# msaad00/agent-bom

Measured on AMD Instinct MI355X. Metric: findings/sec, higher is better.
Workload: dtype fp32; 1 GPU; model=estate-blast-pipeline, global_batch=327063, seq_len=10000000, parallelism=single, nodes_global=11350000, edges_global=18551093, arena_windows=2000000

## Files before the change

agentbom_amd/graph/gpu_engine.py:

```python

from __future__ import annotations

from typing import Optional

import numpy as np

from agentbom_amd.models.blast import HOP_RISK_FACTORS
from agentbom_amd.models.cwe_impact import (
    IMPACT_CODE,
    IMPACT_CREDENTIAL_ACCESS,
    IMPACT_CODE_EXECUTION,
    IMPACT_DATA_LEAK,
    IMPACT_FILE_ACCESS,
    IMPACT_INJECTION,
    IMPACT_SSRF,
)
from agentbom_amd.scan.synth import ET_CONTAINS, ET_HAS_CRED, ET_PROVIDES_TOOL, ET_USES, SyntheticEstate

_FULL_CRED = {IMPACT_CODE[c] for c in (IMPACT_CODE_EXECUTION, IMPACT_CREDENTIAL_ACCESS,
                                       IMPACT_DATA_LEAK, IMPACT_FILE_ACCESS, IMPACT_SSRF)}
_DB_CRED = {IMPACT_CODE[IMPACT_INJECTION]}
_FULL_TOOL = _FULL_CRED
_DB_TOOL = {IMPACT_CODE[IMPACT_INJECTION]}

# ... 179 lines not shown
        raise ValueError("agent index exceeds int32 offsets")
    agent_off = torch.zeros(n_agents + 1, dtype=torch.int64, device=dev)
    torch.cumsum(torch.bincount(key >> 32, minlength=n_agents), 0, out=agent_off[1:])
    return {
        "agent_off": agent_off.to(torch.int32).contiguous(),
        "agent_srv": (key & 0xFFFFFFFF).to(torch.int32).contiguous(),
    }


def blast_index_enabled() -> bool:
    import os

    return os.environ.get("AGENT_BOM_BLAST_INDEX", "1") != "0"


def match_by_window_enabled() -> bool:
    import os

    return os.environ.get("AGENT_BOM_MATCH_BY_WINDOW", "1") != "0"


def findings_native_enabled() -> bool:
    import os

    return os.environ.get("AGENT_BOM_FINDINGS_NATIVE", "1") != "0"


def findings_ahead_enabled() -> bool:
    import os

    return os.environ.get("AGENT_BOM_FINDINGS_AHEAD", "1") != "0"


def expand_dedup_matches(torch, layout: dict, su, sw):
    dev = su.device
    if su.numel() == 0:
        e = torch.empty(0, dtype=torch.int64, device=dev)
        return e, e.clone()
    run_off = layout["run_off"]
    cnt = run_off[su + 1] - run_off[su]
    rep = torch.repeat_interleave(
        torch.arange(su.numel(), device=dev), cnt)
    ends = torch.cumsum(cnt, 0)
    base = torch.cat([torch.zeros(1, dtype=torch.int64, device=dev), ends[:-1]])
    within = torch.arange(int(ends[-1].item()) if ends.numel() else 0,
                          device=dev) - base[rep]
    rows2 = run_off[su][rep] + within
    orig = layout["perm2"][rows2]
    packed = (orig << 32) | sw[rep]
    packed, _ = torch.sort(packed)
    return (packed >> 32), (packed & 0xFFFFFFFF)



_RANK_WS: dict = {}


def rank_order(torch, scores):
    n = scores.numel()
    if n == 0:
        return torch.empty(0, dtype=torch.int64, device=scores.device)
    if scores.is_cuda:
        from agentbom_amd.ops import native

        return native.rank_bucket_order(scores.contiguous(), _RANK_WS)
    q = (scores * 100).round().clamp(0, 1000).to(torch.int64)
# ... 286 lines not shown

    def _blast_counts_join(self, uniq_pkgs):
        torch = self.torch
        n_up = uniq_pkgs.numel()
        pos = torch.arange(n_up, device=self.device)

        srv, carry = self._expand(self.rev, uniq_pkgs, pos, ET_CONTAINS)
        n_servers = self._distinct_counts(carry, srv, n_up)

        ag, carry2 = self._expand(self.rev, srv, carry, ET_USES)
        n_agents = self._distinct_counts(carry2, ag, n_up)

        cr, carry3 = self._expand(self.fwd, srv, carry, ET_HAS_CRED)
        n_creds_all, n_creds_db = self._distinct_counts(
            carry3, cr, n_up, weights=self.node_is_db_cred
        )
        tl, carry4 = self._expand(self.fwd, srv, carry, ET_PROVIDES_TOOL)
        n_tools_all, n_tools_db = self._distinct_counts(
            carry4, tl, n_up, weights=self.node_is_db_tool
        )
        return {
            "uniq_pkgs": uniq_pkgs,
            "n_servers": n_servers,
            "n_agents": n_agents,
            "n_creds_all": n_creds_all,
            "n_creds_db": n_creds_db,
            "n_tools_all": n_tools_all,
            "n_tools_db": n_tools_db,
        }

    def step(self, blast_depth: int = 1, reach_dist=None):
        torch = self.torch
        assembled = None
        if self.use_gpu:
            from agentbom_amd.ops import native

            if self._match_stream is None:
                self._match_stream = torch.cuda.Stream(device=self.device)
            side = self._match_stream
            if reach_dist is None:
                self._reach_begin()
            side.wait_stream(torch.cuda.current_stream())
            dd = self.match_dedup
            with torch.cuda.stream(side):
                if (dd is not None and self.match_table is not None
                        and match_by_window_enabled()):
                    pending = native.match_by_window_launch(
                        self.arena["windows"], self.match_table)
                elif dd is not None:
                    pending = native.match_launch(
                        dd["u_gk"], dd["u_hi"], dd["u_lo"], dd["u_flags"],
                        self.arena["group_keys"], self.arena["group_off"],
                        self.arena["windows"], pkg_win_range=dd["u_ranges"],
                        order=dd["heavy_order"])
                else:
                    pending = native.match_launch(
                        self.pkg_group_key_sorted, self.pkg_key_hi_sorted,
                        self.pkg_key_lo_sorted, self.pkg_flags_sorted,
                        self.arena["group_keys"], self.arena["group_off"],
                        self.arena["windows"], pkg_win_range=self.pkg_win_range)
                counting = None
                if (dd is not None and findings_native_enabled()
                        and self.reach_index is not None and blast_index_enabled()
                        and findings_ahead_enabled()):
                    counting = native.assemble_findings_begin_ahead(
                        pending, dd, self._findings_ws, self.estate.pkg_base,
                        native.blast_inputs(
                            self.rev, self.reach_index, ET_CONTAINS,
                            self.node_is_db_cred, self.node_is_db_tool, self._blast_ws))
                elif dd is not None and findings_native_enabled():
                    counting = native.assemble_findings_begin(
                        pending, dd, self._findings_ws)
            dist = (reach_dist if reach_dist is not None
                    else self.dependency_reach(begun=True))
            torch.cuda.current_stream().wait_stream(side)
            if counting is not None:
                assembled = native.assemble_findings_finish(
                    counting, self.estate.pkg_base)
            else:
                sp, sw = native.match_finalize(pending, sort=False)
                if dd is not None:
                    pkg_idx, win_idx = expand_dedup_matches(torch, dd, sp, sw)
                else:
                    pkg_idx, win_idx = self._unsort_matches(sp, sw)
        else:
            pkg_idx, win_idx = self.match()
            dist = reach_dist if reach_dist is not None else self.dependency_reach()

        if assembled is not None:
            pkg_idx, win_idx = assembled["pkg_idx"], assembled["win_idx"]
            pkg_nodes, pos = assembled["pkg_nodes"], assembled["pos"]
            if "blast_counts" in assembled:
                counts = self._blast_counts_resolve(
                    assembled["uniq_pkgs"], assembled["blast_counts"],
                    assembled["blast_overflow"], assembled["blast_n_overflow"],
                    counts_only=True)
            else:
                counts = self._blast_counts_fused(assembled["uniq_pkgs"],
                                                  assembled["uniq_pkgs32"])
        else:
            pkg_nodes = pkg_idx + self.estate.pkg_base
            counts = self.blast_counts(pkg_nodes)
            pos = torch.searchsorted(counts["uniq_pkgs"], pkg_nodes)
        n_findings = pkg_idx.numel()

        if self.use_gpu:
            from agentbom_amd.ops import native

            scores, n_agents, n_creds, n_tools = native.score_gather(
                win_idx.contiguous(), pkg_nodes.contiguous(), pos.contiguous(),
                self.arena["severity"], self.arena["kev"], self.arena["epss"],
                self.arena["impact"], self.cred_lut, self.tool_lut,
                counts["counts2d"].contiguous(), dist)
        else:
            scores, n_agents, n_creds, n_tools = self._score_cpu(
                counts, pos, pkg_nodes, win_idx, dist)

        res = {
            "n_findings": int(n_findings),
            "scores": scores,
            "order": rank_order(torch, scores),
            "pkg_idx": pkg_idx,
            "win_idx": win_idx,
            "n_agents": n_agents,
            "n_creds": n_creds,
            "n_tools": n_tools,
            "reach_dist": dist,
        }
        if blast_depth > 1:
            hops = self._blast_hops(
                counts["uniq_pkgs"],
                assembled["uniq_pkgs32"] if assembled is not None else None, blast_depth)
            hop_depth = hops["hop_depth"][pos]
            res["hop_depth"] = hop_depth
            res["transitive_agents"] = hops["t_agents"][pos]
            res["transitive_creds"] = hops["t_creds"][pos]
            res["transitive_scores"] = torch.where(
                hop_depth > 1, scores * self._hop_factor[hop_depth.to(torch.int64)],
                torch.zeros_like(scores))
        return res

    def _blast_hops(self, uniq_pkgs, uniq_pkgs32, max_depth: int) -> dict:
        torch = self.torch
        if self.use_gpu:
            from agentbom_amd.ops import native

            if uniq_pkgs32 is None:
                uniq_pkgs32 = uniq_pkgs.to(torch.int32).contiguous()
            out = native.blast_hops(uniq_pkgs32, self.rev, self.reach_index, self.agent_index,
                                    ET_CONTAINS, max_depth, self._hops_ws)
        else:
            from agentbom_amd.ops import cpu_ref

            hop_agents, t_creds, hop_depth = cpu_ref.blast_hops(
# ... 402 lines not shown
```

agentbom_amd/ops/csrc/abom_api.h:

```cpp
#pragma once

#ifdef __cplusplus
extern "C" {
#endif

int abom_abi_version();
int abom_device_count();
const char* abom_error_string(int code);

int abom_match(
    const void* pkg_group_key, const void* pkg_key_hi, const void* pkg_key_lo,
    const void* pkg_flags, long long num_packages,
    const void* group_keys, const void* group_off, long long num_groups,
    const void* w_intro_hi, const void* w_intro_lo, const void* w_fixed_hi, const void* w_fixed_lo,
    const void* w_last_hi, const void* w_last_lo, const void* w_flags, const void* w_packed,
    const void* pkg_wbeg, const void* pkg_wend, const void* p_order,
    void* out_pairs, void* out_count, long long capacity, void* stream);
int abom_match_by_window(
    const void* w_intro_hi, const void* w_intro_lo, const void* w_fixed_hi, const void* w_fixed_lo,
    const void* w_last_hi, const void* w_last_lo, const void* w_flags,
    const void* w_rbeg, const void* w_rend, long long num_windows,
    const void* s_key, const void* s_row,
    void* out_pairs, void* out_count, long long capacity, void* stream);
int abom_match_by_window_tiled(
// ... 46 lines not shown
    long long num_nodes, void* dist, unsigned int cur_level, const void* first_parent,
    void* next_count, void* open_count, void* stream);
int abom_bfs_run_indexed(
    const void* row_off, const void* col, const void* etype, unsigned int allowed_mask,
    const void* sources, long long n_sources, void* dist, long long num_nodes,
    void* frontier_a, void* frontier_b, void* heavy_queue, void* counters,
    int max_levels, const void* edge_src, long long num_edges,
    const void* rev_off, const void* rev_col, const void* rev_et, const void* first_parent,
    int begun, long long sources_degree, void* host_counters, void* stream);

int abom_reach_hops(
    const void* row_off, const void* col, const void* etype, unsigned int allowed_mask,
    const void* sources, int n_sources, int words, long long num_nodes,
    const void* target_slot, void* hops, long long hops_stride, long long col_base,
    int max_depth,
    void* seen, void* cur, void* nxt, void* queue_a, void* queue_b, void* heavy_queue,
    void* counters, void* host_counters, void* stream);

int abom_impact_query(
    const void* row_off, const void* col, const void* etype, unsigned int allowed_mask,
    const void* query_sources, int num_queries, int max_hops, int max_nodes_per_query,
    void* out_nodes, void* out_hops, void* out_counts, void* out_truncated, void* stream);

int abom_risk_score(
    const void* severity, const void* n_agents, const void* n_creds, const void* n_tools,
    const void* flags, const void* epss, const void* scorecard, const void* reach,
    void* out, long long n, const float* weights22, void* stream);
int abom_score_gather(
    const void* win_idx, const void* pkg_nodes, const void* pos,
    const void* a_sev, const void* a_kev, const void* a_epss, const void* a_impact,
    const void* cred_lut, const void* tool_lut, const void* counts2d,
    const void* dist, void* out_scores, void* out_agents, void* out_creds,
    void* out_tools, long long n, const float* weights22, void* stream);
int abom_severity_histogram(
    const void* owner, const void* severity, void* hist, long long n, void* stream);

int abom_blast_counts(
    const void* pkgs, long long n,
    const void* rev_off, const void* rev_col, const void* rev_et,
    const void* fwd_off, const void* fwd_col, const void* fwd_et,
    int et_contains, int et_uses, int et_cred, int et_tool,
    const void* node_is_db_cred, const void* node_is_db_tool,
    void* out_counts, void* out_overflow, void* stream);
int abom_blast_counts_indexed(
    const void* pkgs, long long n,
    const void* rev_off, const void* rev_col, const void* rev_et, int et_contains,
    const void* reach_off, const void* reach_col, const void* reach_db,
    long long row_base, long long num_rows,
    const void* node_is_db_cred, const void* node_is_db_tool,
    void* queue, void* counters, void* out_counts, void* out_overflow, void* stream);
int abom_blast_counts_indexed_sized(
    const void* pkgs, const void* n_dev, long long n_cap,
    const void* rev_off, const void* rev_col, const void* rev_et, int et_contains,
    const void* reach_off, const void* reach_col, const void* reach_db,
    long long row_base, long long num_rows,
    const void* node_is_db_cred, const void* node_is_db_tool,
    void* queue, void* counters, void* host_counters,
    void* out_counts, void* out_overflow, void* stream);

int abom_blast_hops_cap(int which);
int abom_blast_hops(
    const void* pkgs, long long n,
    const void* rev_off, const void* rev_col, const void* rev_et, int et_contains,
    const void* reach_off, const void* reach_col, long long row_base, long long num_rows,
    const void* agent_off, const void* agent_srv, long long num_agents, int max_depth,
    void* queue, void* counters,
    void* out_hop_agents, void* out_creds, void* out_depth, void* out_overflow, void* stream);
int abom_blast_hops_sized(
    const void* pkgs, const void* n_dev, long long n_cap,
    const void* rev_off, const void* rev_col, const void* rev_et, int et_contains,
    const void* reach_off, const void* reach_col, long long row_base, long long num_rows,
    const void* agent_off, const void* agent_srv, long long num_agents, int max_depth,
    void* queue, void* counters, void* host_counters,
    void* out_hop_agents, void* out_creds, void* out_depth, void* out_overflow, void* stream);

int abom_path_relax(
    const void* edge_src, const void* col, const void* etype, const void* edge_weight,
    const void* cur, void* nxt, const void* node_boost, const void* etype_boost,
    const void* etype_trav, const void* etype_gate, const void* node_gate,
    long long num_edges, void* stream);

int abom_rank_order(
    const void* scores, long long n, void* hist, void* bin_scratch, int nblocks,
    void* order, void* stream);

int abom_findings_count(
    const void* pairs, const void* count, long long capacity,
    const void* run_off, const void* perm2, const void* row_of,
    long long num_rows, long long num_packages,
    void* bitmap, void* row_cnt, void* row_tail, void* chain_prev,
    void* rank_of, void* word_f, void* block_sums, void* totals, void* stream);
int abom_findings_emit(
    const void* pairs, const void* count, long long capacity,
    const void* row_of, long long num_rows, long long num_packages,
    void* bitmap, void* row_cnt, void* row_tail, const void* chain_prev,
    const void* rank_of, const void* word_f, const void* block_off,
    long long pkg_base, long long num_findings, long long num_unique,
    void* out_pkg_idx, void* out_win_idx, void* out_pkg_nodes, void* out_pos,
    void* out_uniq64, void* out_uniq32, void* stream);
int abom_findings_emit_sized(
    const void* pairs, const void* count, long long capacity,
    const void* row_of, long long num_rows, long long num_packages,
    void* bitmap, void* row_cnt, void* row_tail, const void* chain_prev,
    const void* rank_of, const void* word_f, const void* block_off,
    long long pkg_base, const void* totals, long long findings_cap, long long unique_cap,
    void* num_sized,
    void* out_pkg_idx, void* out_win_idx, void* out_pkg_nodes, void* out_pos,
    void* out_uniq64, void* out_uniq32, void* stream);
int abom_findings_ahead(
    const void* pairs, const void* count, long long capacity,
    const void* run_off, const void* perm2, const void* row_of,
    long long num_rows, long long num_packages,
    void* bitmap, void* row_cnt, void* row_tail, void* chain_prev,
    void* rank_of, void* word_f, void* block_sums, void* totals, void* host_totals,
    long long pkg_base, long long findings_cap, long long unique_cap, void* num_sized,
    void* out_pkg_idx, void* out_win_idx, void* out_pkg_nodes, void* out_pos,
    void* out_uniq64, void* out_uniq32,
// ... 33 lines not shown
```

agentbom_amd/ops/csrc/abom_common.h:

```cpp
#pragma once

#include <hip/hip_runtime.h>
#include <stdint.h>

#define ABOM_UNVISITED 0xFFFFFFFFu

namespace abom {

__device__ __forceinline__ bool key_lt(uint64_t ahi, uint64_t alo, uint64_t bhi, uint64_t blo) {
    return (ahi < bhi) | ((ahi == bhi) & (alo < blo));
}
__device__ __forceinline__ bool key_ge(uint64_t ahi, uint64_t alo, uint64_t bhi, uint64_t blo) {
    return !key_lt(ahi, alo, bhi, blo);
}
__device__ __forceinline__ bool key_gt(uint64_t ahi, uint64_t alo, uint64_t bhi, uint64_t blo) {
    return key_lt(bhi, blo, ahi, alo);
}

__device__ __forceinline__ bool edge_filtered(const uint8_t* __restrict__ etype,
                                              uint32_t allowed_mask, uint64_t e) {
    return etype && !((allowed_mask >> etype[e]) & 1u);
}

constexpr uint8_t WF_HAS_INTRO = 1u << 0;
constexpr uint8_t WF_HAS_FIXED = 1u << 1;
constexpr uint8_t WF_HAS_LAST = 1u << 2;
constexpr uint8_t WF_CPU_FALLBACK = 1u << 3;
constexpr uint8_t WF_UNFIXED_SUPPRESSED = 1u << 4;

constexpr uint8_t PF_ENCODABLE = 1u << 0;

inline int grid_for(long long work, int block) {
    long long blocks = (work + block - 1) / block;
    if (blocks > 2048) blocks = 2048;
    if (blocks < 1) blocks = 1;
    return (int)blocks;
}

}

#define ABOM_CHECK(expr)                                                     \
    do {                                                                     \
        hipError_t _e = (expr);                                              \
        if (_e != hipSuccess) return (int)_e;                                \
    } while (0)
```

agentbom_amd/ops/csrc/rank.hip:

```cpp
#include "abom_api.h"
#include "abom_wave.h"

namespace {

constexpr int RANK_BINS = 1024;
constexpr int RANK_CHUNK = 256;

__device__ __forceinline__ int score_bin(float s) {
    float q = rintf(s * 100.0f);
    q = fminf(fmaxf(q, 0.0f), 1000.0f);
    return 1000 - (int)q;
}

__device__ __forceinline__ uint64_t eq_group(int bin, uint64_t act) {
    uint64_t m = act;
    #pragma unroll
    for (int b = 0; b < 10; ++b) {
        uint64_t bb = __ballot((bin >> b) & 1);
        m &= ((bin >> b) & 1) ? bb : ~bb;
    }
    return m;
}

__global__ void rank_hist_kernel(const float* __restrict__ scores,
                                 long long n,
                                 int* __restrict__ hist ) {
    __shared__ int lhist[RANK_BINS];
    const int lane = threadIdx.x;
    for (int i = lane; i < RANK_BINS; i += 64) lhist[i] = 0;
    __syncthreads();
    const long long base = (long long)blockIdx.x * RANK_CHUNK;
    for (int r = 0; r < RANK_CHUNK; r += 64) {
        const long long idx = base + r + lane;
        const bool active = idx < n;
        const int bin = active ? score_bin(scores[idx]) : 0;
        const uint64_t act = __ballot(active);
        const uint64_t eq = eq_group(bin, act);
        if (active && (eq & ((1ull << lane) - 1)) == 0)
            lhist[bin] += __popcll(eq);
    }
    __syncthreads();
    int* gh = hist + (long long)blockIdx.x * RANK_BINS;
    for (int i = lane; i < RANK_BINS; i += 64) gh[i] = lhist[i];
}

__global__ void rank_scan_blocks_kernel(int* __restrict__ hist,
                                        int nblocks,
                                        int* __restrict__ bin_total) {
    const int bin = blockIdx.x;
    const int lane = threadIdx.x;
    int carry = 0;
    for (int t = 0; t < nblocks; t += 64) {
        const int idx = t + lane;
        const int v = (idx < nblocks)
            ? hist[(long long)idx * RANK_BINS + bin] : 0;
        int total;
        const int before = abom::wave_exclusive_scan(v, lane, &total);
        if (idx < nblocks)
            hist[(long long)idx * RANK_BINS + bin] = before + carry;
        carry += total;
    }
    if (lane == 0) bin_total[bin] = carry;
}

__global__ void rank_scan_bins_kernel(int* __restrict__ bin_total,
                                      int* __restrict__ bin_base) {
    __shared__ int vals[RANK_BINS];
    const int lane = threadIdx.x;
    for (int i = lane; i < RANK_BINS; i += 64) vals[i] = bin_total[i];
    __syncthreads();
    if (lane == 0) {
        int acc = 0;
        for (int i = 0; i < RANK_BINS; ++i) {
            const int v = vals[i];
            vals[i] = acc;
            acc += v;
        }
    }
    __syncthreads();
    for (int i = lane; i < RANK_BINS; i += 64) bin_base[i] = vals[i];
}

__global__ void rank_scatter_kernel(const float* __restrict__ scores,
                                    long long n,
                                    const int* __restrict__ hist,
                                    const int* __restrict__ bin_base,
                                    long long* __restrict__ order) {
    __shared__ int run[RANK_BINS];
    const int lane = threadIdx.x;
    for (int i = lane; i < RANK_BINS; i += 64) run[i] = 0;
    __syncthreads();
    const long long base = (long long)blockIdx.x * RANK_CHUNK;
    const int* gb = hist + (long long)blockIdx.x * RANK_BINS;
    for (int r = 0; r < RANK_CHUNK; r += 64) {
        const long long idx = base + r + lane;
        const bool active = idx < n;
        const int bin = active ? score_bin(scores[idx]) : 0;
        const uint64_t act = __ballot(active);
        const uint64_t eq = eq_group(bin, act);
        if (active) {
            const uint64_t lower = eq & ((1ull << lane) - 1);
            const long long pos =
                (long long)bin_base[bin] + gb[bin] + run[bin] + __popcll(lower);
            order[pos] = idx;
            if (lower == 0)
                run[bin] += __popcll(eq);
        }
    }
}

}

extern "C" int abom_rank_order(const void* scores, long long n,
                               void* hist, void* bin_scratch, int nblocks,
                               void* order, void* stream) {
    if (n <= 0) return 0;
    hipStream_t s = (hipStream_t)stream;
    int* bin_total = (int*)bin_scratch;
    int* bin_base = bin_total + RANK_BINS;
    hipLaunchKernelGGL(rank_hist_kernel, dim3(nblocks), dim3(64), 0, s,
                       (const float*)scores, n, (int*)hist);
    hipLaunchKernelGGL(rank_scan_blocks_kernel, dim3(RANK_BINS), dim3(64), 0, s,
                       (int*)hist, nblocks, bin_total);
    hipLaunchKernelGGL(rank_scan_bins_kernel, dim3(1), dim3(64), 0, s,
                       bin_total, bin_base);
    hipLaunchKernelGGL(rank_scatter_kernel, dim3(nblocks), dim3(64), 0, s,
                       (const float*)scores, n, (const int*)hist,
                       (const int*)bin_base, (long long*)order);
    return (int)hipGetLastError();
}
```

agentbom_amd/ops/csrc/score.hip:

```cpp

#include <string.h>

#include "abom_api.h"
#include "abom_common.h"

namespace abom {


struct RiskWeights {
    float base_critical, base_high, base_medium, base_low;
    float agent_w, agent_cap, cred_w, cred_cap, tool_w, tool_cap;
    float ai_boost, kev_boost, epss_boost, epss_threshold;
    float sc_t1, sc_b1, sc_t2, sc_b2, sc_t3, sc_b3;
    float reach_boost, unreach_penalty;
};

static RiskWeights load_weights(const float* weights22) {
    static_assert(sizeof(RiskWeights) == 22 * sizeof(float), "RiskWeights is 22 packed floats");
    RiskWeights w;
    memcpy(&w, weights22, sizeof(w));
    return w;
}

__device__ __forceinline__ float score_one(
// ... 37 lines not shown
    const uint8_t* __restrict__ a_impact,
    const uint8_t* __restrict__ cred_lut,
    const uint8_t* __restrict__ tool_lut,
    const int* __restrict__ counts2d,
    const uint32_t* __restrict__ dist,
    float* __restrict__ out_scores,
    int* __restrict__ out_agents,
    int* __restrict__ out_creds,
    int* __restrict__ out_tools,
    long long n, RiskWeights w) {
    const long long stride = (long long)gridDim.x * blockDim.x;
    for (long long i = (long long)blockIdx.x * blockDim.x + threadIdx.x; i < n; i += stride) {
        const long long wrow = win_idx[i];
        const long long crow = pos[i] * 6;
        const uint8_t impact = a_impact[wrow];
        const uint8_t ccls = cred_lut[impact];
        const uint8_t tcls = tool_lut[impact];
        const int n_creds = ccls == 2 ? counts2d[crow + 2]
                          : ccls == 1 ? counts2d[crow + 3] : 0;
        const int n_tools = tcls == 2 ? counts2d[crow + 4]
                          : tcls == 1 ? counts2d[crow + 5] : 0;
        const int n_agents = counts2d[crow + 1];
        const uint8_t flags = (uint8_t)(a_kev[wrow] ? 2u : 0u);
        const int8_t reach = dist[pkg_nodes[i]] != ABOM_UNVISITED ? 1 : 0;
        out_scores[i] = score_one(a_sev[wrow], (uint32_t)n_agents,
                                  (uint32_t)n_creds, (uint32_t)n_tools, flags,
                                  a_epss[wrow], -1.0f, reach, w);
        out_agents[i] = n_agents;
        out_creds[i] = n_creds;
        out_tools[i] = n_tools;
    }
}

__global__ void risk_score_kernel(
    const uint8_t* __restrict__ severity,
    const uint32_t* __restrict__ n_agents,
    const uint32_t* __restrict__ n_creds,
    const uint32_t* __restrict__ n_tools,
    const uint8_t* __restrict__ flags,
    const float* __restrict__ epss,
    const float* __restrict__ scorecard,
    const int8_t* __restrict__ reach,
    float* __restrict__ out,
    long long n, RiskWeights w) {
    const long long stride = (long long)gridDim.x * blockDim.x;
    for (long long i = (long long)blockIdx.x * blockDim.x + threadIdx.x; i < n; i += stride) {
        out[i] = score_one(severity[i], n_agents[i], n_creds[i], n_tools[i],
                           flags[i], epss[i], scorecard[i], reach[i], w);
    }
}

__global__ void severity_histogram_kernel(
    const uint32_t* __restrict__ owner,
    const uint8_t* __restrict__ severity,
    unsigned int* __restrict__ hist,
    long long n) {
    const long long stride = (long long)gridDim.x * blockDim.x;
    for (long long i = (long long)blockIdx.x * blockDim.x + threadIdx.x; i < n; i += stride) {
        atomicAdd(&hist[(long long)owner[i] * 6 + severity[i]], 1u);
    }
}

}

extern "C" int abom_risk_score(
    const void* severity, const void* n_agents, const void* n_creds, const void* n_tools,
    const void* flags, const void* epss, const void* scorecard, const void* reach,
    void* out, long long n, const float* weights22, void* stream) {
    const int block = 256;
    hipLaunchKernelGGL(abom::risk_score_kernel, dim3(abom::grid_for(n, block)), dim3(block), 0,
                       (hipStream_t)stream, (const uint8_t*)severity, (const uint32_t*)n_agents,
                       (const uint32_t*)n_creds, (const uint32_t*)n_tools, (const uint8_t*)flags,
                       (const float*)epss, (const float*)scorecard, (const int8_t*)reach,
                       (float*)out, n, abom::load_weights(weights22));
    return (int)hipGetLastError();
}

extern "C" int abom_score_gather(
    const void* win_idx, const void* pkg_nodes, const void* pos,
    const void* a_sev, const void* a_kev, const void* a_epss, const void* a_impact,
    const void* cred_lut, const void* tool_lut, const void* counts2d,
    const void* dist, void* out_scores, void* out_agents, void* out_creds,
    void* out_tools, long long n, const float* weights22, void* stream) {
    const int block = 256;
    hipLaunchKernelGGL(abom::score_gather_kernel, dim3(abom::grid_for(n, block)),
                       dim3(block), 0, (hipStream_t)stream,
                       (const long long*)win_idx, (const long long*)pkg_nodes,
                       (const long long*)pos, (const uint8_t*)a_sev,
                       (const uint8_t*)a_kev, (const float*)a_epss,
                       (const uint8_t*)a_impact, (const uint8_t*)cred_lut,
                       (const uint8_t*)tool_lut, (const int*)counts2d,
                       (const uint32_t*)dist, (float*)out_scores,
                       (int*)out_agents, (int*)out_creds, (int*)out_tools, n,
                       abom::load_weights(weights22));
    return (int)hipGetLastError();
}

extern "C" int abom_severity_histogram(
    const void* owner, const void* severity, void* hist, long long n, void* stream) {
    const int block = 256;
    hipLaunchKernelGGL(abom::severity_histogram_kernel, dim3(abom::grid_for(n, block)),
                       dim3(block), 0, (hipStream_t)stream, (const uint32_t*)owner,
                       (const uint8_t*)severity, (unsigned int*)hist, n);
    return (int)hipGetLastError();
}
```

agentbom_amd/ops/native.py:

```python

from __future__ import annotations

import ctypes
import os
from pathlib import Path
from typing import Optional

import numpy as np

_SO_PATH = Path(__file__).resolve().parent / "_abom_gpu.so"
_lib: Optional[ctypes.CDLL] = None

_c = ctypes.c_void_p
_i64 = ctypes.c_longlong
_u32 = ctypes.c_uint
_i32 = ctypes.c_int
_f64 = ctypes.c_double
_fp = ctypes.POINTER(ctypes.c_float)

_SIGNATURES = {
    "abom_abi_version": ([], _i32),
    "abom_device_count": ([], _i32),
    "abom_error_string": ([_i32], ctypes.c_char_p),
    "abom_match": ([
# ... 72 lines not shown
    ], _i32),
    "abom_bfs_run_indexed": ([
        _c, _c, _c, _u32,
        _c, _i64, _c, _i64,
        _c, _c, _c, _c,
        _i32, _c, _i64,
        _c, _c, _c, _c,
        _i32, _i64, _c, _c,
    ], _i32),
    "abom_reach_hops": ([
        _c, _c, _c, _u32,
        _c, _i32, _i32, _i64,
        _c, _c, _i64, _i64,
        _i32,
        _c, _c, _c, _c, _c, _c,
        _c, _c, _c,
    ], _i32),
    "abom_impact_query": ([
        _c, _c, _c, _u32,
        _c, _i32, _i32, _i32,
        _c, _c, _c, _c, _c,
    ], _i32),
    "abom_risk_score": ([
        _c, _c, _c, _c,
        _c, _c, _c, _c,
        _c, _i64, _fp, _c,
    ], _i32),
    "abom_score_gather": ([
        _c, _c, _c,
        _c, _c, _c, _c,
        _c, _c, _c,
        _c, _c, _c, _c,
        _c, _i64, _fp, _c,
    ], _i32),
    "abom_severity_histogram": ([_c, _c, _c, _i64, _c], _i32),
    "abom_blast_counts": ([
        _c, _i64,
        _c, _c, _c,
        _c, _c, _c,
        _i32, _i32, _i32, _i32,
        _c, _c,
        _c, _c, _c,
    ], _i32),
    "abom_blast_counts_indexed": ([
        _c, _i64,
        _c, _c, _c, _i32,
        _c, _c, _c,
        _i64, _i64,
        _c, _c,
        _c, _c, _c, _c, _c,
    ], _i32),
    "abom_blast_counts_indexed_sized": ([
        _c, _c, _i64,
        _c, _c, _c, _i32,
        _c, _c, _c,
        _i64, _i64,
        _c, _c,
        _c, _c, _c,
        _c, _c, _c,
    ], _i32),
    "abom_blast_hops_cap": ([_i32], _i32),
    "abom_blast_hops": ([
        _c, _i64,
        _c, _c, _c, _i32,
        _c, _c, _i64, _i64,
        _c, _c, _i64, _i32,
        _c, _c,
        _c, _c, _c, _c, _c,
    ], _i32),
    "abom_blast_hops_sized": ([
        _c, _c, _i64,
        _c, _c, _c, _i32,
        _c, _c, _i64, _i64,
        _c, _c, _i64, _i32,
        _c, _c, _c,
        _c, _c, _c, _c, _c,
    ], _i32),
    "abom_path_relax": ([
        _c, _c, _c, _c,
        _c, _c, _c, _c,
        _c, _c, _c,
        _i64, _c,
    ], _i32),
    "abom_rank_order": ([
        _c, _i64, _c, _c, _i32,
        _c, _c,
    ], _i32),
    "abom_findings_count": ([
        _c, _c, _i64,
        _c, _c, _c,
        _i64, _i64,
        _c, _c, _c, _c,
        _c, _c, _c, _c, _c,
    ], _i32),
    "abom_findings_emit": ([
        _c, _c, _i64,
        _c, _i64, _i64,
        _c, _c, _c, _c,
        _c, _c, _c,
        _i64, _i64, _i64,
        _c, _c, _c, _c,
        _c, _c, _c,
    ], _i32),
    "abom_findings_emit_sized": ([
        _c, _c, _i64,
        _c, _i64, _i64,
        _c, _c, _c, _c,
        _c, _c, _c,
        _i64, _c, _i64, _i64,
        _c,
        _c, _c, _c, _c,
        _c, _c, _c,
    ], _i32),
    "abom_findings_ahead": ([
        _c, _c, _i64,
        _c, _c, _c,
        _i64, _i64,
        _c, _c, _c, _c,
        _c, _c, _c, _c, _c,
# ... 326 lines not shown
    counts, uniq32 = blob32[:6 * NU_cap], blob32[6 * NU_cap:7 * NU_cap]
    overflow = blob32[7 * NU_cap:].view(torch.uint8)
    fresh.extend((blob64, blob32))
    for key, numel in (("queue", NU_cap), ("counters", 2)):
        before = bws.get(key)
        if _buf(bws, key, numel, torch.int32, dev) is not before:
            fresh.append(bws[key])
    host_counters = _blast_host_counters(bws)
    bitmap, row_cnt, row_tail, chain_prev, rank_of, word_f, block_sums = state["bufs"]
    totals = state["totals"]
    rev, index = blast["rev"], blast["index"]
    rc = lib.abom_findings_ahead(
        _ptr(pairs), _ptr(count), cap,
        _ptr(layout["run_off"]), _ptr(layout["perm2"]), _ptr(layout["row_of"]),
        state["U"], state["P"],
        _ptr(bitmap), _ptr(row_cnt), _ptr(row_tail), _ptr(chain_prev),
        _ptr(rank_of), _ptr(word_f), _ptr(block_sums), _ptr(totals),
        _ptr(ws["fa_host_totals"]),
        int(pkg_base), F_cap, NU_cap, ctypes.c_void_p(totals.data_ptr() + 24),
        _ptr(out64[0]), _ptr(out64[1]), _ptr(out64[2]), _ptr(out64[3]),
        _ptr(uniq64), _ptr(uniq32),
        _ptr(rev["row_off"]), _ptr(rev["col"]), _ptr(rev["etype"]), blast["et_contains"],
        _ptr(index["reach_off"]), _ptr(index["reach_col"]), _ptr(index["reach_db"]),
        index["row_base"], index["reach_off"].shape[0],
        _ptr(blast["node_is_db_cred"]), _ptr(blast["node_is_db_tool"]),
        _ptr(bws["queue"]), _ptr(bws["counters"]), _ptr(host_counters),
        _ptr(counts), _ptr(overflow), _stream(),
    )
    _check(rc, "abom_findings_ahead")
    ws["fa_counted"].record()
    state["ahead"].update(caps=(F_cap, NU_cap), outs=(out64, uniq64, uniq32, counts, overflow),
                          host_counters=host_counters)
    return state


def _finish_ahead(state: dict, out: dict) -> dict:
    ahead = state.get("ahead")
    if ahead is None:
        return out
    b = ahead["blast"]
    counts, overflow, n_overflow = blast_counts_indexed(
        out["uniq_pkgs32"], b["rev"], b["index"], b["et_contains"],
        b["node_is_db_cred"], b["node_is_db_tool"], b["ws"])
    out.update(blast_counts=counts, blast_overflow=overflow, blast_n_overflow=n_overflow)
    state["ws"]["fa_ahead_hit"] = False
    state["ws"]["fa_ahead_cap"] = (findings_ahead_capacity(out["pkg_idx"].numel()),
                                   findings_ahead_capacity(out["uniq_pkgs"].numel()))
    return out


def assemble_findings_finish(state: dict, pkg_base: int) -> dict:
    import torch

    lib = load()
    pending, layout, ws, cap = state["pending"], state["layout"], state["ws"], state["cap"]
    pairs, count = pending["out_pairs"], pending["out_count"]
    dev = pairs.device
    if state["bufs"] is None:
        e64 = [torch.empty(0, dtype=torch.int64, device=dev) for _ in range(5)]
        return _finish_ahead(state, dict(
            zip(("pkg_idx", "win_idx", "pkg_nodes", "pos", "uniq_pkgs"), e64),
            uniq_pkgs32=torch.empty(0, dtype=torch.int32, device=dev)))
    cur = torch.cuda.current_stream()
    if cur != state["stream"]:
        for t in state["fresh"]:
            t.record_stream(cur)
# ... 674 lines not shown
        _ptr(edge_src), _ptr(col), _ptr(etype),
        _ptr(edge_weight) if edge_weight is not None else None,
        _ptr(cur), _ptr(nxt), _ptr(node_boost), _ptr(etype_boost),
        _ptr(etype_trav), _ptr(etype_gate),
        _ptr(node_gate) if node_gate is not None else None,
        etype.numel(), _stream(),
    )
    _check(rc, "abom_path_relax")


_RANK_BINS = 1024
_RANK_CHUNK = 256


def rank_bucket_order(scores, workspace: Optional[dict] = None):
    import torch

    lib = load()
    n = scores.numel()
    dev = scores.device
    if n == 0:
        return torch.empty(0, dtype=torch.int64, device=dev)
    nblocks = (n + _RANK_CHUNK - 1) // _RANK_CHUNK
    ws = workspace if workspace is not None else {}
    hist = _buf(ws, "rank_hist", nblocks * _RANK_BINS, torch.int32, dev)
    scratch = _buf(ws, "rank_scratch", 2 * _RANK_BINS, torch.int32, dev)
    order = torch.empty(n, dtype=torch.int64, device=dev)
    rc = lib.abom_rank_order(_ptr(scores), n, _ptr(hist), _ptr(scratch),
                             nblocks, _ptr(order), _stream())
    _check(rc, "abom_rank_order")
    return order




def _heavy_rows(row_off):
    import torch

    deg = row_off[1:] - row_off[:-1]
    return torch.nonzero(deg >= CENTRALITY_HEAVY_DEGREE).flatten().to(torch.int32)


def pagerank(rev_off, rev_col, out_degree, num_nodes: int, damping: float = 0.85,
             iterations: int = 50, workspace: Optional[dict] = None):
    import torch

    lib = load()
    dev = rev_off.device
    if num_nodes == 0:
        return torch.empty(0, dtype=torch.float64, device=dev)
    ws = workspace if workspace is not None else {}
    rank_a = _buf(ws, "pr_rank_a", num_nodes, torch.float64, dev)
    rank_b = _buf(ws, "pr_rank_b", num_nodes, torch.float64, dev)
    contrib_a = _buf(ws, "pr_contrib_a", num_nodes, torch.float64, dev)
    contrib_b = _buf(ws, "pr_contrib_b", num_nodes, torch.float64, dev)
    partials = _buf(ws, "pr_partials", 2 * _PAGERANK_PARTIALS, torch.float64, dev)
    scalars = _buf(ws, "pr_scalars", 2, torch.float64, dev)
    heavy = _heavy_rows(rev_off)
    rc = lib.abom_pagerank_run(
        _ptr(rev_off), _ptr(rev_col), _ptr(heavy), heavy.numel(),
        _ptr(out_degree), num_nodes, float(damping), PAGERANK_TOLERANCE,
        int(iterations), _ptr(rank_a), _ptr(rank_b), _ptr(contrib_a), _ptr(contrib_b),
        _ptr(partials), _ptr(scalars), _stream(),
    )
    if rc < 0:
        _check(-rc, "abom_pagerank_run")
# ... 144 lines not shown
```

Measured before the change: 523.7 million findings/s.

## Launch score and rank kernels speculatively before findings finish using device-side counts

Adds sized variants of the score-gather and radix rank kernels that read the finding count from device memory, gated by device flags. When findings are assembled ahead, scoring and ranking are enqueued before the host syncs on the finish step. The results are kept only if the ahead path hit and there was no blast overflow. This aims to overlap the tail work with the host round-trip and avoid a sync-bound launch sequence. The cost is wasted GPU work on a miss, plus kernels launched at capacity size that exit early.

```diff
diff --git a/agentbom_amd/graph/gpu_engine.py b/agentbom_amd/graph/gpu_engine.py
--- a/agentbom_amd/graph/gpu_engine.py
+++ b/agentbom_amd/graph/gpu_engine.py
@@ -235,6 +235,12 @@
     return os.environ.get("AGENT_BOM_FINDINGS_AHEAD", "1") != "0"
 
 
+def tail_ahead_enabled() -> bool:
+    import os
+
+    return os.environ.get("AGENT_BOM_TAIL_AHEAD", "1") != "0"
+
+
 def expand_dedup_matches(torch, layout: dict, su, sw):
     dev = su.device
     if su.numel() == 0:
@@ -587,6 +593,7 @@
     def step(self, blast_depth: int = 1, reach_dist=None):
         torch = self.torch
         assembled = None
+        tail = None
         if self.use_gpu:
             from agentbom_amd.ops import native
 
@@ -629,6 +636,15 @@
             dist = (reach_dist if reach_dist is not None
                     else self.dependency_reach(begun=True))
             torch.cuda.current_stream().wait_stream(side)
+            if counting is not None and tail_ahead_enabled():
+                bufs = native.findings_ahead_buffers(counting)
+                if bufs is not None and dist.dtype == torch.int32 and dist.is_contiguous():
+                    tail = native.score_rank_sized(
+                        bufs["win_idx"], bufs["pkg_nodes"], bufs["pos"],
+                        self.arena["severity"], self.arena["kev"], self.arena["epss"],
+                        self.arena["impact"], self.cred_lut, self.tool_lut,
+                        bufs["counts"], dist, bufs["n_dev"], bufs["F_cap"],
+                        gate=bufs["gate"], workspace=_RANK_WS)
             if counting is not None:
                 assembled = native.assemble_findings_finish(
                     counting, self.estate.pkg_base)
@@ -659,7 +675,16 @@
             pos = torch.searchsorted(counts["uniq_pkgs"], pkg_nodes)
         n_findings = pkg_idx.numel()
 
-        if self.use_gpu:
+        order = None
+        if tail is not None:
+            self._findings_ws["tail_ahead_hit"] = bool(
+                self._findings_ws.get("fa_ahead_hit")
+                and assembled.get("blast_n_overflow") == 0)
+            if not self._findings_ws["tail_ahead_hit"]:
+                tail = None
+        if tail is not None:
+            scores, n_agents, n_creds, n_tools, order = (t[:n_findings] for t in tail)
+        elif self.use_gpu:
             from agentbom_amd.ops import native
 
             scores, n_agents, n_creds, n_tools = native.score_gather(
@@ -674,7 +699,7 @@
         res = {
             "n_findings": int(n_findings),
             "scores": scores,
-            "order": rank_order(torch, scores),
+            "order": order if order is not None else rank_order(torch, scores),
             "pkg_idx": pkg_idx,
             "win_idx": win_idx,
             "n_agents": n_agents,
diff --git a/agentbom_amd/ops/csrc/abom_api.h b/agentbom_amd/ops/csrc/abom_api.h
--- a/agentbom_amd/ops/csrc/abom_api.h
+++ b/agentbom_amd/ops/csrc/abom_api.h
@@ -102,6 +102,13 @@
     const void* cred_lut, const void* tool_lut, const void* counts2d,
     const void* dist, void* out_scores, void* out_agents, void* out_creds,
     void* out_tools, long long n, const float* weights22, void* stream);
+int abom_score_gather_sized(
+    const void* win_idx, const void* pkg_nodes, const void* pos,
+    const void* a_sev, const void* a_kev, const void* a_epss, const void* a_impact,
+    const void* cred_lut, const void* tool_lut, const void* counts2d,
+    const void* dist, void* out_scores, void* out_agents, void* out_creds,
+    void* out_tools, const void* n_dev, long long n_cap, const void* gate,
+    const void* skip, const float* weights22, void* stream);
 int abom_severity_histogram(
     const void* owner, const void* severity, void* hist, long long n, void* stream);
 
@@ -153,6 +160,19 @@
 int abom_rank_order(
     const void* scores, long long n, void* hist, void* bin_scratch, int nblocks,
     void* order, void* stream);
+int abom_rank_order_sized(
+    const void* scores, const void* n_dev, long long n_cap,
+    const void* gate, const void* skip,
+    void* hist, void* bin_scratch,
+    void* order, void* stream);
+int abom_score_rank_sized(
+    const void* win_idx, const void* pkg_nodes, const void* pos,
+    const void* a_sev, const void* a_kev, const void* a_epss, const void* a_impact,
+    const void* cred_lut, const void* tool_lut, const void* counts2d,
+    const void* dist, void* out_scores, void* out_agents, void* out_creds,
+    void* out_tools, const void* n_dev, long long n_cap, const void* gate,
+    const void* skip, const float* weights22,
+    void* hist, void* bin_scratch, void* order, void* stream);
 
 int abom_findings_count(
     const void* pairs, const void* count, long long capacity,
diff --git a/agentbom_amd/ops/csrc/abom_common.h b/agentbom_amd/ops/csrc/abom_common.h
--- a/agentbom_amd/ops/csrc/abom_common.h
+++ b/agentbom_amd/ops/csrc/abom_common.h
@@ -30,6 +30,15 @@
 
 constexpr uint8_t PF_ENCODABLE = 1u << 0;
 
+__device__ __forceinline__ long long sized_count(const long long* n_dev, long long n_cap,
+                                                 const long long* gate,
+                                                 const unsigned int* skip) {
+    if (skip && *skip != 0) return 0;
+    if (gate && *gate == 0) return 0;
+    const long long n = *n_dev;
+    return (n < 0 || n > n_cap) ? 0 : n;
+}
+
 inline int grid_for(long long work, int block) {
     long long blocks = (work + block - 1) / block;
     if (blocks > 2048) blocks = 2048;
diff --git a/agentbom_amd/ops/csrc/rank.hip b/agentbom_amd/ops/csrc/rank.hip
--- a/agentbom_amd/ops/csrc/rank.hip
+++ b/agentbom_amd/ops/csrc/rank.hip
@@ -22,10 +22,10 @@
     return m;
 }
 
-__global__ void rank_hist_kernel(const float* __restrict__ scores,
-                                 long long n,
-                                 int* __restrict__ hist ) {
-    __shared__ int lhist[RANK_BINS];
+__device__ __forceinline__ void rank_hist_block(const float* __restrict__ scores,
+                                                long long n,
+                                                int* __restrict__ hist ,
+                                                int* lhist) {
     const int lane = threadIdx.x;
     for (int i = lane; i < RANK_BINS; i += 64) lhist[i] = 0;
     __syncthreads();
@@ -44,9 +44,27 @@
     for (int i = lane; i < RANK_BINS; i += 64) gh[i] = lhist[i];
 }
 
-__global__ void rank_scan_blocks_kernel(int* __restrict__ hist,
-                                        int nblocks,
-                                        int* __restrict__ bin_total) {
+__global__ void rank_hist_kernel(const float* __restrict__ scores,
+                                 long long n,
+                                 int* __restrict__ hist) {
+    __shared__ int lhist[RANK_BINS];
+    rank_hist_block(scores, n, hist, lhist);
+}
+
+__global__ void rank_hist_sized_kernel(const float* __restrict__ scores,
+                                       const long long* __restrict__ n_dev, long long n_cap,
+                                       const long long* __restrict__ gate,
+                                       const unsigned int* __restrict__ skip,
+                                       int* __restrict__ hist) {
+    __shared__ int lhist[RANK_BINS];
+    const long long n = abom::sized_count(n_dev, n_cap, gate, skip);
+    if ((long long)blockIdx.x * RANK_CHUNK >= n) return;
+    rank_hist_block(scores, n, hist, lhist);
+}
+
+__device__ __forceinline__ void rank_scan_blocks_bin(int* __restrict__ hist,
+                                                     int nblocks,
+                                                     int* __restrict__ bin_total) {
     const int bin = blockIdx.x;
     const int lane = threadIdx.x;
     int carry = 0;
@@ -63,6 +81,22 @@
     if (lane == 0) bin_total[bin] = carry;
 }
 
+__global__ void rank_scan_blocks_kernel(int* __restrict__ hist,
+                                        int nblocks,
+                                        int* __restrict__ bin_total) {
+    rank_scan_blocks_bin(hist, nblocks, bin_total);
+}
+
+__global__ void rank_scan_blocks_sized_kernel(int* __restrict__ hist,
+                                              const long long* __restrict__ n_dev,
+                                              long long n_cap,
+                                              const long long* __restrict__ gate,
+                                              const unsigned int* __restrict__ skip,
+                                              int* __restrict__ bin_total) {
+    const long long n = abom::sized_count(n_dev, n_cap, gate, skip);
+    rank_scan_blocks_bin(hist, (int)((n + RANK_CHUNK - 1) / RANK_CHUNK), bin_total);
+}
+
 __global__ void rank_scan_bins_kernel(int* __restrict__ bin_total,
                                       int* __restrict__ bin_base) {
     __shared__ int vals[RANK_BINS];
@@ -81,12 +115,12 @@
     for (int i = lane; i < RANK_BINS; i += 64) bin_base[i] = vals[i];
 }
 
-__global__ void rank_scatter_kernel(const float* __restrict__ scores,
-                                    long long n,
-                                    const int* __restrict__ hist,
-                                    const int* __restrict__ bin_base,
-                                    long long* __restrict__ order) {
-    __shared__ int run[RANK_BINS];
+__device__ __forceinline__ void rank_scatter_block(const float* __restrict__ scores,
+                                                   long long n,
+                                                   const int* __restrict__ hist,
+                                                   const int* __restrict__ bin_base,
+                                                   long long* __restrict__ order,
+                                                   int* run) {
     const int lane = threadIdx.x;
     for (int i = lane; i < RANK_BINS; i += 64) run[i] = 0;
     __syncthreads();
@@ -107,6 +141,29 @@
                 run[bin] += __popcll(eq);
         }
     }
+}
+
+__global__ void rank_scatter_kernel(const float* __restrict__ scores,
+                                    long long n,
+                                    const int* __restrict__ hist,
+                                    const int* __restrict__ bin_base,
+                                    long long* __restrict__ order) {
+    __shared__ int run[RANK_BINS];
+    rank_scatter_block(scores, n, hist, bin_base, order, run);
+}
+
+__global__ void rank_scatter_sized_kernel(const float* __restrict__ scores,
+                                          const long long* __restrict__ n_dev,
+                                          long long n_cap,
+                                          const long long* __restrict__ gate,
+                                          const unsigned int* __restrict__ skip,
+                                          const int* __restrict__ hist,
+                                          const int* __restrict__ bin_base,
+                                          long long* __restrict__ order) {
+    __shared__ int run[RANK_BINS];
+    const long long n = abom::sized_count(n_dev, n_cap, gate, skip);
+    if ((long long)blockIdx.x * RANK_CHUNK >= n) return;
+    rank_scatter_block(scores, n, hist, bin_base, order, run);
 }
 
 }
@@ -129,3 +186,45 @@
                        (const int*)bin_base, (long long*)order);
     return (int)hipGetLastError();
 }
+
+extern "C" int abom_rank_order_sized(const void* scores, const void* n_dev, long long n_cap,
+                                     const void* gate, const void* skip,
+                                     void* hist, void* bin_scratch,
+                                     void* order, void* stream) {
+    if (n_cap < 0 || n_cap >= (1ll << 31) || !n_dev) return (int)hipErrorInvalidValue;
+    if (n_cap == 0) return 0;
+    hipStream_t s = (hipStream_t)stream;
+    const int nblocks = (int)((n_cap + RANK_CHUNK - 1) / RANK_CHUNK);
+    const long long* nd = (const long long*)n_dev;
+    const long long* g = (const long long*)gate;
+    const unsigned int* sk = (const unsigned int*)skip;
+    int* bin_total = (int*)bin_scratch;
+    int* bin_base = bin_total + RANK_BINS;
+    hipLaunchKernelGGL(rank_hist_sized_kernel, dim3(nblocks), dim3(64), 0, s,
+                       (const float*)scores, nd, n_cap, g, sk, (int*)hist);
+    hipLaunchKernelGGL(rank_scan_blocks_sized_kernel, dim3(RANK_BINS), dim3(64), 0, s,
+                       (int*)hist, nd, n_cap, g, sk, bin_total);
+    hipLaunchKernelGGL(rank_scan_bins_kernel, dim3(1), dim3(64), 0, s,
+                       bin_total, bin_base);
+    hipLaunchKernelGGL(rank_scatter_sized_kernel, dim3(nblocks), dim3(64), 0, s,
+                       (const float*)scores, nd, n_cap, g, sk, (const int*)hist,
+                       (const int*)bin_base, (long long*)order);
+    return (int)hipGetLastError();
+}
+
+extern "C" int abom_score_rank_sized(
+    const void* win_idx, const void* pkg_nodes, const void* pos,
+    const void* a_sev, const void* a_kev, const void* a_epss, const void* a_impact,
+    const void* cred_lut, const void* tool_lut, const void* counts2d,
+    const void* dist, void* out_scores, void* out_agents, void* out_creds,
+    void* out_tools, const void* n_dev, long long n_cap, const void* gate,
+    const void* skip, const float* weights22,
+    void* hist, void* bin_scratch, void* order, void* stream) {
+    int rc = abom_score_gather_sized(win_idx, pkg_nodes, pos, a_sev, a_kev, a_epss, a_impact,
+                                     cred_lut, tool_lut, counts2d, dist, out_scores,
+                                     out_agents, out_creds, out_tools, n_dev, n_cap, gate,
+                                     skip, weights22, stream);
+    if (rc) return rc;
+    return abom_rank_order_sized(out_scores, n_dev, n_cap, gate, skip, hist, bin_scratch,
+                                 order, stream);
+}
diff --git a/agentbom_amd/ops/csrc/score.hip b/agentbom_amd/ops/csrc/score.hip
--- a/agentbom_amd/ops/csrc/score.hip
+++ b/agentbom_amd/ops/csrc/score.hip
@@ -93,6 +93,49 @@
     }
 }
 
+__global__ void score_gather_sized_kernel(
+    const long long* __restrict__ win_idx,
+    const long long* __restrict__ pkg_nodes,
+    const long long* __restrict__ pos,
+    const uint8_t* __restrict__ a_sev,
+    const uint8_t* __restrict__ a_kev,
+    const float* __restrict__ a_epss,
+    const uint8_t* __restrict__ a_impact,
+    const uint8_t* __restrict__ cred_lut,
+    const uint8_t* __restrict__ tool_lut,
+    const int* __restrict__ counts2d,
+    const uint32_t* __restrict__ dist,
+    float* __restrict__ out_scores,
+    int* __restrict__ out_agents,
+    int* __restrict__ out_creds,
+    int* __restrict__ out_tools,
+    const long long* __restrict__ n_dev, long long n_cap,
+    const long long* __restrict__ gate, const unsigned int* __restrict__ skip,
+    RiskWeights w) {
+    const long long n = sized_count(n_dev, n_cap, gate, skip);
+    const long long stride = (long long)gridDim.x * blockDim.x;
+    for (long long i = (long long)blockIdx.x * blockDim.x + threadIdx.x; i < n; i += stride) {
+        const long long wrow = win_idx[i];
+        const long long crow = pos[i] * 6;
+        const uint8_t impact = a_impact[wrow];
+        const uint8_t ccls = cred_lut[impact];
+        const uint8_t tcls = tool_lut[impact];
+        const int n_creds = ccls == 2 ? counts2d[crow + 2]
+                          : ccls == 1 ? counts2d[crow + 3] : 0;
+        const int n_tools = tcls == 2 ? counts2d[crow + 4]
+                          : tcls == 1 ? counts2d[crow + 5] : 0;
+        const int n_agents = counts2d[crow + 1];
+        const uint8_t flags = (uint8_t)(a_kev[wrow] ? 2u : 0u);
+        const int8_t reach = dist[pkg_nodes[i]] != ABOM_UNVISITED ? 1 : 0;
+        out_scores[i] = score_one(a_sev[wrow], (uint32_t)n_agents,
+                                  (uint32_t)n_creds, (uint32_t)n_tools, flags,
+                                  a_epss[wrow], -1.0f, reach, w);
+        out_agents[i] = n_agents;
+        out_creds[i] = n_creds;
+        out_tools[i] = n_tools;
+    }
+}
+
 __global__ void risk_score_kernel(
     const uint8_t* __restrict__ severity,
     const uint32_t* __restrict__ n_agents,
@@ -157,6 +200,30 @@
     return (int)hipGetLastError();
 }
 
+extern "C" int abom_score_gather_sized(
+    const void* win_idx, const void* pkg_nodes, const void* pos,
+    const void* a_sev, const void* a_kev, const void* a_epss, const void* a_impact,
+    const void* cred_lut, const void* tool_lut, const void* counts2d,
+    const void* dist, void* out_scores, void* out_agents, void* out_creds,
+    void* out_tools, const void* n_dev, long long n_cap, const void* gate,
+    const void* skip, const float* weights22, void* stream) {
+    if (n_cap < 0 || !n_dev) return (int)hipErrorInvalidValue;
+    if (n_cap == 0) return 0;
+    const int block = 256;
+    hipLaunchKernelGGL(abom::score_gather_sized_kernel, dim3(abom::grid_for(n_cap, block)),
+                       dim3(block), 0, (hipStream_t)stream,
+                       (const long long*)win_idx, (const long long*)pkg_nodes,
+                       (const long long*)pos, (const uint8_t*)a_sev,
+                       (const uint8_t*)a_kev, (const float*)a_epss,
+                       (const uint8_t*)a_impact, (const uint8_t*)cred_lut,
+                       (const uint8_t*)tool_lut, (const int*)counts2d,
+                       (const uint32_t*)dist, (float*)out_scores,
+                       (int*)out_agents, (int*)out_creds, (int*)out_tools,
+                       (const long long*)n_dev, n_cap, (const long long*)gate,
+                       (const unsigned int*)skip, abom::load_weights(weights22));
+    return (int)hipGetLastError();
+}
+
 extern "C" int abom_severity_histogram(
     const void* owner, const void* severity, void* hist, long long n, void* stream) {
     const int block = 256;
diff --git a/agentbom_amd/ops/native.py b/agentbom_amd/ops/native.py
--- a/agentbom_amd/ops/native.py
+++ b/agentbom_amd/ops/native.py
@@ -128,6 +128,14 @@
         _c, _c, _c,
         _c, _c, _c, _c,
         _c, _i64, _fp, _c,
+    ], _i32),
+    "abom_score_gather_sized": ([
+        _c, _c, _c,
+        _c, _c, _c, _c,
+        _c, _c, _c,
+        _c, _c, _c, _c,
+        _c, _c, _i64, _c,
+        _c, _fp, _c,
     ], _i32),
     "abom_severity_histogram": ([_c, _c, _c, _i64, _c], _i32),
     "abom_blast_counts": ([
@@ -181,6 +189,21 @@
     "abom_rank_order": ([
         _c, _i64, _c, _c, _i32,
         _c, _c,
+    ], _i32),
+    "abom_rank_order_sized": ([
+        _c, _c, _i64,
+        _c, _c,
+        _c, _c,
+        _c, _c,
+    ], _i32),
+    "abom_score_rank_sized": ([
+        _c, _c, _c,
+        _c, _c, _c, _c,
+        _c, _c, _c,
+        _c, _c, _c, _c,
+        _c, _c, _i64, _c,
+        _c, _fp,
+        _c, _c, _c, _c,
     ], _i32),
     "abom_findings_count": ([
         _c, _c, _i64,
@@ -573,6 +596,16 @@
     state["ahead"].update(caps=(F_cap, NU_cap), outs=(out64, uniq64, uniq32, counts, overflow),
                           host_counters=host_counters)
     return state
+
+
+def findings_ahead_buffers(state: dict) -> Optional[dict]:
+    ahead = state.get("ahead")
+    if state["bufs"] is None or ahead is None or ahead["caps"] is None:
+        return None
+    out64, _uniq64, _uniq32, counts, _overflow = ahead["outs"]
+    totals = state["totals"]
+    return {"win_idx": out64[1], "pkg_nodes": out64[2], "pos": out64[3], "counts": counts,
+            "n_dev": totals[0:1], "gate": totals[3:4], "F_cap": ahead["caps"][0]}
 
 
 def _finish_ahead(state: dict, out: dict) -> dict:
@@ -1313,6 +1346,47 @@
     return order
 
 
+def score_rank_sized(win_idx, pkg_nodes, pos, arena_sev, arena_kev, arena_epss,
+                     arena_impact, cred_lut, tool_lut, counts2d, dist, n_dev, n_cap: int,
+                     gate=None, skip=None, workspace: Optional[dict] = None):
+    import torch
+
+    lib = load()
+    n_cap = int(n_cap)
+    dev = win_idx.device
+    if min(win_idx.numel(), pkg_nodes.numel(), pos.numel()) < n_cap:
+        raise ValueError("score_rank_sized: an input holds fewer than n_cap elements")
+    for name, t, dtype in (("win_idx", win_idx, torch.int64), ("pkg_nodes", pkg_nodes, torch.int64),
+                           ("pos", pos, torch.int64), ("counts2d", counts2d, torch.int32),
+                           ("dist", dist, torch.int32), ("n_dev", n_dev, torch.int64)):
+        if t.dtype != dtype or not t.is_contiguous():
+            raise ValueError(f"score_rank_sized: {name} must be contiguous {dtype}, "
+                             f"got {t.dtype}, contiguous={t.is_contiguous()}")
+    blob32 = torch.empty(4 * n_cap, dtype=torch.int32, device=dev)
+    order = torch.empty(n_cap, dtype=torch.int64, device=dev)
+    scores = blob32[:n_cap].view(torch.float32)
+    out_agents, out_creds, out_tools = (blob32[k * n_cap:(k + 1) * n_cap] for k in (1, 2, 3))
+    if n_cap == 0:
+        return scores, out_agents, out_creds, out_tools, order
+    nblocks = (n_cap + _RANK_CHUNK - 1) // _RANK_CHUNK
+    ws = workspace if workspace is not None else {}
+    hist = _buf(ws, "rank_hist", nblocks * _RANK_BINS, torch.int32, dev)
+    scratch = _buf(ws, "rank_scratch", 2 * _RANK_BINS, torch.int32, dev)
+    w = risk_weights_array()
+    rc = lib.abom_score_rank_sized(
+        _ptr(win_idx), _ptr(pkg_nodes), _ptr(pos), _ptr(arena_sev),
+        _ptr(arena_kev), _ptr(arena_epss), _ptr(arena_impact), _ptr(cred_lut),
+        _ptr(tool_lut), _ptr(counts2d), _ptr(dist), _ptr(scores),
+        _ptr(out_agents), _ptr(out_creds), _ptr(out_tools), _ptr(n_dev), n_cap,
+        _ptr(gate) if gate is not None else None,
+        _ptr(skip) if skip is not None else None,
+        w.ctypes.data_as(ctypes.POINTER(ctypes.c_float)),
+        _ptr(hist), _ptr(scratch), _ptr(order), _stream(),
+    )
+    _check(rc, "abom_score_rank_sized")
+    return scores, out_agents, out_creds, out_tools, order
+
+
 
 
 def _heavy_rows(row_off):
```

Result: faster. 549.9 million findings/s (median of 6 runs) (+5.0%).
